# tugitbartlomiej/ViTParticleFilterTracker

Measured on AMD Instinct MI355X. Metric: frames/sec @ 4096 particles, ViT-B/16 224px; 1/2/4/8 MI355X scaling, higher is better.
Workload: dtype bf16; 1 GPU; 4096 particles, vit_base_patch16_224 bf16, 224x224 frames, full tracking step per frame; particles=4096, particles_per_gpu=4096, arch=vit_base_patch16_224, hip_graph=True, parallelism=particle-shard x1

## Files before the change

### include/vpf.h

```cpp
#ifndef VPF_H
#define VPF_H
#include <stddef.h>
#include <stdint.h>

#ifdef __cplusplus
extern "C" {
#endif

#define VPF_ERR_ARG (-1)

#define VPF_EPI_BIAS 0
#define VPF_EPI_BIAS_GELU 1
#define VPF_EPI_BIAS_RESIDUAL 2
#define VPF_EPI_PATCH 3
#define VPF_EPI_LN 4
#define VPF_EPI_LN_GELU 5

const char* vpf_version(void);

int vpf_predict(float* particles, int64_t n, int64_t ld, int64_t global_begin, uint64_t seed,
                uint32_t frame, float sig_x, float sig_y, float sig_s, float width, float height,
                float smin, float smax, void* stream);

int vpf_crop_patches_bf16(const uint8_t* frame, int H, int W, uint32_t* rgba_ws, const float* particles,
                          int64_t ld, int64_t n, float w0, float h0, int S, int patch, int Kp,
                          const float* norm_ab_host, uint16_t* out, void* stream);
int vpf_crop_patches_f32(const uint8_t* frame, int H, int W, uint32_t* rgba_ws, const float* particles,
                         int64_t ld, int64_t n, float w0, float h0, int S, int patch, int Kp,
                         const float* norm_ab_host, float* out, void* stream);

int vpf_cls_rows_bf16(uint16_t* tokens, int64_t n_part, int N, int D, const float* cls,
                      const float* pos, float* stats_out, int parts, void* stream);
int vpf_cls_rows_f32(float* tokens, int64_t n_part, int N, int D, const float* cls, const float* pos,
                     void* stream);

int vpf_gemm_bf16(const uint16_t* A, int64_t lda, const uint16_t* W, const float* bias,
                  const uint16_t* residual, const float* pos, int patch_rows, const float* row_stats,
                  const float* colsum, uint16_t* C, int64_t ldc, int64_t M, int64_t N, int64_t K,
                  int epilogue, int stats_parts, float ln_eps, float* stats_out, uint8_t* C8, int64_t ld8,
                  uint32_t* Cs, int64_t lds_c, void* stream);
int vpf_gemm_bf16_splitk(const uint16_t* A, int64_t lda, const uint16_t* W, const float* bias,
                         const uint16_t* residual, const float* row_stats, const float* colsum, uint16_t* C,
                         int64_t ldc, int64_t M, int64_t N, int64_t K, int epilogue, int splits, float* stats_out,
                         float* partial_ws, int64_t ws_elems, void* stream);
int vpf_gemm_tune(int kernel, int group);

int vpf_gemm_mx8(const uint8_t* A8, int64_t lda, const uint32_t* As, int64_t lds_a, const uint8_t* W8,
                 const uint32_t* Ws, const float* bias, const uint16_t* residual, const float* row_stats,
                 const float* colsum, uint16_t* C, int64_t ldc, uint8_t* C8, int64_t ld8, uint32_t* Cs,
                 int64_t lds_c, int64_t M, int64_t N, int64_t K, int epilogue, int stats_parts, float ln_eps,
                 float* stats_out, void* stream);
int vpf_quantize_mx8(const uint16_t* X, int64_t ldx, int64_t rows, int64_t K, int64_t out_stride, uint8_t* X8,
                     int64_t ld8, uint32_t* S, int64_t lds, void* stream);
int vpf_gemm_f32(const float* A, int64_t lda, const float* W, const float* bias, const float* residual,
                 const float* pos, int patch_rows, const float* row_stats, const float* colsum, float* C,
                 int64_t ldc, int64_t M, int64_t N, int64_t K, int epilogue, void* stream);

int vpf_row_stats_bf16(const uint16_t* x, int64_t rows, int D, int64_t x_stride, float eps, float* out,
                       void* stream);
int vpf_row_stats_f32(const float* x, int64_t rows, int D, int64_t x_stride, float eps, float* out,
                      void* stream);

int vpf_stats_combine(const float* planes, int parts, int64_t plane_stride, int64_t rows, int D, float eps, float* out,
                      void* stream);

int vpf_layernorm_bf16(const uint16_t* x, int64_t rows, int D, int64_t x_stride, const float* gamma,
                       const float* beta, float eps, uint16_t* y, int64_t y_stride, void* stream);
int vpf_layernorm_f32(const float* x, int64_t rows, int D, int64_t x_stride, const float* gamma,
                      const float* beta, float eps, float* y, int64_t y_stride, void* stream);

int vpf_attention_bf16(const uint16_t* qkv, uint16_t* out, int64_t B, int N, int H, int hd,
                       float scale, int q_rows, void* stream);
int vpf_attention_bf16_mx8(const uint16_t* qkv, int64_t B, int N, int H, int hd, float scale, uint8_t* out8,
                           int64_t ld8, uint32_t* s8, int64_t lds, void* stream);
int vpf_attention_f32(const float* qkv, float* out, int64_t B, int N, int H, int hd, float scale,
                      int q_rows, void* stream);
int vpf_head_gather_bf16(const uint16_t* Y, int64_t n, int H, int hd, uint16_t* out, int64_t ldo, void* stream);
int vpf_cls_attn_fold_bf16(const uint16_t* tokens, int64_t n_part, int N, int H, const float* planes,
                           int64_t plane_rows, float eps, const uint16_t* G, int64_t ldg, const uint16_t* q,
                           int64_t ldq, const float* bk, float scale, uint16_t* out, int64_t ldo, void* stream);

int vpf_cls_weight_bf16(const uint16_t* tokens, int64_t n, int N, int D, const float* gamma,
                        const float* beta, float eps, const float* tmpl, float lam, int bits,
                        float* feat_out, float* sim_out, int64_t* Q, void* stream);
int vpf_cls_weight_f32(const float* tokens, int64_t n, int N, int D, const float* gamma,
                       const float* beta, float eps, const float* tmpl, float lam, int bits,
                       float* feat_out, float* sim_out, int64_t* Q, void* stream);

int vpf_cosine_weight_f32(const float* feat, int64_t n, int D, const float* tmpl, float lam, int bits,
                          float* sim_out, int64_t* Q, void* stream);

int vpf_shard_stats(const int64_t* Q, const float* particles, int64_t ld, int64_t n, int64_t* out_T,
                    double* out_sums, void* stream);

int vpf_resample(const int64_t* Q, int64_t n_local, int64_t global_begin, int64_t offset,
                 int64_t total, int64_t P, uint32_t U, int uniform, int64_t slot_begin,
                 int64_t slot_end, const float* particles, int64_t ld, int32_t* anc_out,
                 float* states_out, int64_t out_ld, int64_t* cdf_ws, void* stream);

int vpf_estimate_resample(const int64_t* Q, int64_t q_stride, const float* particles, int64_t ld,
                          int64_t p_stride, int64_t n_shard, int64_t P, uint64_t seed, uint32_t frame,
                          int64_t slot_begin, int64_t slot_end, int32_t* anc_out, float* states_out,
                          int64_t out_ld, int64_t* cdf_ws, int64_t* stats_out, void* stream);

#define VPF_RESAMPLE_SYSTEMATIC 0
#define VPF_RESAMPLE_STRATIFIED 1

int vpf_weight_prior(int64_t* Q, const int64_t* carry, int64_t n, int bits, void* stream);

int vpf_estimate_resample_ex(const int64_t* Q, int64_t q_stride, const float* particles, int64_t ld,
                             int64_t p_stride, int64_t n_shard, int64_t P, uint64_t seed, uint32_t frame,
                             int64_t slot_begin, int64_t slot_end, int32_t* anc_out, float* states_out,
                             int64_t out_ld, int64_t* cdf_ws, int64_t* stats_out, int method, double ess_tau,
                             int bits, int64_t* carry_out, void* stream);

#ifdef __cplusplus
}
#endif
#endif
```

### vitparticlefiltertracker_amd/_lib.py

```python
from __future__ import annotations

import ctypes
import os
import subprocess
import threading

import torch

_HERE = os.path.dirname(os.path.abspath(__file__))
LIB_PATH = os.environ.get("VPF_LIB_PATH") or os.path.join(_HERE, "libvpf.so")
CSRC = os.path.join(_HERE, "csrc")

_lock = threading.Lock()
_lib = None

VPF_EPI_BIAS = 0
VPF_EPI_BIAS_GELU = 1
VPF_EPI_BIAS_RESIDUAL = 2
VPF_EPI_PATCH = 3
VPF_EPI_LN = 4
VPF_EPI_LN_GELU = 5
VPF_RESAMPLE_SYSTEMATIC = 0
VPF_RESAMPLE_STRATIFIED = 1

_P, _I64, _I32, _U64, _U32, _F32, _F64 = (ctypes.c_void_p, ctypes.c_int64, ctypes.c_int, ctypes.c_uint64,
                                          ctypes.c_uint32, ctypes.c_float, ctypes.c_double)

SIGNATURES = {
    "vpf_predict": [_P, _I64, _I64, _I64, _U64, _U32, _F32, _F32, _F32, _F32, _F32, _F32, _F32, _P],
    "vpf_crop_patches_bf16": [_P, _I32, _I32, _P, _P, _I64, _I64, _F32, _F32, _I32, _I32, _I32, _P, _P, _P],
    "vpf_crop_patches_f32": [_P, _I32, _I32, _P, _P, _I64, _I64, _F32, _F32, _I32, _I32, _I32, _P, _P, _P],
    "vpf_cls_rows_bf16": [_P, _I64, _I32, _I32, _P, _P, _P, _I32, _P],
    "vpf_cls_rows_f32": [_P, _I64, _I32, _I32, _P, _P, _P],
    "vpf_gemm_bf16": [_P, _I64, _P, _P, _P, _P, _I32, _P, _P, _P, _I64, _I64, _I64, _I64, _I32, _I32, _F32, _P,
                      _P, _I64, _P, _I64, _P],
    "vpf_gemm_mx8": [_P, _I64, _P, _I64, _P, _P, _P, _P, _P, _P, _P, _I64, _P, _I64, _P, _I64, _I64, _I64, _I64,
                     _I32, _I32, _F32, _P, _P],
    "vpf_quantize_mx8": [_P, _I64, _I64, _I64, _I64, _P, _I64, _P, _I64, _P],
    "vpf_gemm_bf16_splitk": [_P, _I64, _P, _P, _P, _P, _P, _P, _I64, _I64, _I64, _I64, _I32, _I32, _P, _P, _I64, _P],
    "vpf_gemm_tune": [_I32, _I32],
    "vpf_gemm_f32": [_P, _I64, _P, _P, _P, _P, _I32, _P, _P, _P, _I64, _I64, _I64, _I64, _I32, _P],
    "vpf_row_stats_bf16": [_P, _I64, _I32, _I64, _F32, _P, _P],
    "vpf_stats_combine": [_P, _I32, _I64, _I64, _I32, _F32, _P, _P],
    "vpf_row_stats_f32": [_P, _I64, _I32, _I64, _F32, _P, _P],
    "vpf_layernorm_bf16": [_P, _I64, _I32, _I64, _P, _P, _F32, _P, _I64, _P],
    "vpf_layernorm_f32": [_P, _I64, _I32, _I64, _P, _P, _F32, _P, _I64, _P],
    "vpf_attention_bf16": [_P, _P, _I64, _I32, _I32, _I32, _F32, _I32, _P],
    "vpf_attention_f32": [_P, _P, _I64, _I32, _I32, _I32, _F32, _I32, _P],
    "vpf_attention_bf16_mx8": [_P, _I64, _I32, _I32, _I32, _F32, _P, _I64, _P, _I64, _P],
    "vpf_head_gather_bf16": [_P, _I64, _I32, _I32, _P, _I64, _P],
    "vpf_cls_attn_fold_bf16": [_P, _I64, _I32, _I32, _P, _I64, _F32, _P, _I64, _P, _I64, _P, _F32, _P, _I64, _P],
    "vpf_cls_weight_bf16": [_P, _I64, _I32, _I32, _P, _P, _F32, _P, _F32, _I32, _P, _P, _P, _P],
    "vpf_cls_weight_f32": [_P, _I64, _I32, _I32, _P, _P, _F32, _P, _F32, _I32, _P, _P, _P, _P],
    "vpf_cosine_weight_f32": [_P, _I64, _I32, _P, _F32, _I32, _P, _P, _P],
    "vpf_shard_stats": [_P, _P, _I64, _I64, _P, _P, _P],
    "vpf_resample": [_P, _I64, _I64, _I64, _I64, _I64, _U32, _I32, _I64, _I64, _P, _I64, _P, _P, _I64, _P, _P],
    "vpf_estimate_resample": [_P, _I64, _P, _I64, _I64, _I64, _I64, _U64, _U32, _I64, _I64, _P, _P, _I64, _P, _P,
                              _P],
    "vpf_weight_prior": [_P, _P, _I64, _I32, _P],
    "vpf_estimate_resample_ex": [_P, _I64, _P, _I64, _I64, _I64, _I64, _U64, _U32, _I64, _I64, _P, _P, _I64, _P, _P,
                                 _I32, _F64, _I32, _P, _P],
}


class VPFError(RuntimeError):
    pass


def build(force: bool = False) -> str:
    args = ["make", "-s", "-C", CSRC, "-j8"]
    if force:
        subprocess.run(["make", "-s", "-C", CSRC, "clean"], check=True)
    subprocess.run(args, check=True)
    return LIB_PATH


def lib() -> ctypes.CDLL:
    global _lib
    if _lib is not None:
        return _lib
    with _lock:
        if _lib is None:
            if not os.path.exists(LIB_PATH):
                raise VPFError(f"libvpf.so not found at {LIB_PATH}; run `python -c 'import __graft_entry__ as g; "
                               f"g.build()'` (or `make -C {CSRC}`)")
            L = ctypes.CDLL(LIB_PATH, mode=ctypes.RTLD_GLOBAL)
            override = os.environ.get("VPF_LIB_PATH") is not None
            for name, argtypes in SIGNATURES.items():
                if override and not hasattr(L, name):
                    continue
                fn = getattr(L, name)
                fn.argtypes = argtypes
                fn.restype = ctypes.c_int
            L.vpf_version.argtypes = []
            L.vpf_version.restype = ctypes.c_char_p
            _lib = L
    return _lib


def check(rc: int, name: str) -> None:
    if rc != 0:
        if rc == -1:
            raise VPFError(f"{name}: argument violates the shape contract of include/vpf.h")
        raise VPFError(f"{name}: HIP error {rc}")


def stream_ptr(stream=None) -> int:
    s = stream if stream is not None else torch.cuda.current_stream()
    return s.cuda_stream


def ptr(t) -> int:
    return 0 if t is None else t.data_ptr()


def call(name: str, *args) -> None:
    check(getattr(lib(), name)(*args), name)
```

### vitparticlefiltertracker_amd/csrc/gemm_bf16.hip

```cpp
#include <algorithm>
#include "gemm_common.h"

using namespace vpf;
using namespace vpf::gemm;

namespace {

constexpr int BK = 64;
constexpr int OPERAND_BYTES = BM * BK * 2;
static_assert(OPERAND_BYTES == TILE_BYTES, "bf16 K-tile geometry");
constexpr int AUX_PARTS = 15;
constexpr int MAX_PARTS = 16;
constexpr int AUX_BYTES = 2048 + AUX_PARTS * 2048;

template <int EPI, bool WIDE = false, bool OUT8 = false, bool PART = false>
__global__ __launch_bounds__(NTHREADS) void k_gemm_bf16(const bf16_t* __restrict__ A, int lda,
                                                        const bf16_t* __restrict__ W,
                                                        const float* __restrict__ bias,
                                                        const bf16_t* residual,
                                                        const float* __restrict__ pos, int g2,
                                                        const float2* __restrict__ stats,
                                                        const float* __restrict__ colsum,
                                                        bf16_t* C, int ldc, int M, int N, int K, int group,
                                                        int stats_parts, float ln_eps, float* stats_out,
                                                        int stats_rows, Out8 o8) {
    constexpr int SMEM = 5 * OPERAND_BYTES;
    static_assert(AUX_BYTES <= OPERAND_BYTES, "aux region must fit the free A slot of the deep ring");
    __shared__ __attribute__((aligned(16))) char smem[SMEM];
    const int tid = threadIdx.x, lane = tid & 63;
    const int wid = __builtin_amdgcn_readfirstlane(tid >> 6);

    int m0, n0;
    tile_of(M, N, group, m0, n0);
    constexpr bool DIRECT = (EPI == VPF_EPI_LN_GELU || EPI == VPF_EPI_BIAS_GELU) && !OUT8 && !PART;

    const int kbase = PART ? (int)blockIdx.y * (K / (int)gridDim.y) : 0;
    const char* Ablk = reinterpret_cast<const char*>(A) + (size_t)m0 * lda * 2 + (size_t)kbase * 2;
    const char* Bblk = reinterpret_cast<const char*>(W) + (size_t)n0 * K * 2 + (size_t)kbase * 2;
    uint32_t offA[4], offB[4];
#pragma unroll
    for (int i = 0; i < 4; ++i) {
        const int g = i * 8 + wid;
        const int row = 8 * g + (lane >> 3);
        const int pch = lane & 7;
        const int lch = pch ^ ((row >> 1) & 7);
        const int ra = min(row, M - 1 - m0);
        const int rb = min(DIRECT ? wperm(row) : row, N - 1 - n0);
        offA[i] = (uint32_t)ra * (uint32_t)(lda * 2) + (uint32_t)(lch * 16);
        offB[i] = (uint32_t)rb * (uint32_t)(K * 2) + (uint32_t)(lch * 16);
    }
    auto stage_a = [&](int kt) {
        char* la = smem + (kt % 3) * OPERAND_BYTES;
        const uint32_t koff = (uint32_t)kt * (BK * 2);
#pragma unroll
        for (int i = 0; i < 4; ++i)
            __builtin_amdgcn_global_load_lds((gptr_t)(Ablk + offA[i] + koff), (lptr_t)(la + (i * 8 + wid) * 1024), 16, 0, 0);
    };
    auto stage_b = [&](int kt) {
        char* lb = smem + (3 + (kt & 1)) * OPERAND_BYTES;
        const uint32_t koff = (uint32_t)kt * (BK * 2);
#pragma unroll
        for (int i = 0; i < 4; ++i)
            __builtin_amdgcn_global_load_lds((gptr_t)(Bblk + offB[i] + koff), (lptr_t)(lb + (i * 8 + wid) * 1024), 16, 0, 0);
    };

    const int wm = wid >> 2, wn = wid & 3;
    f32x4 acc[4][8];
#pragma unroll
    for (int j = 0; j < 4; ++j)
#pragma unroll
        for (int i = 0; i < 8; ++i) acc[j][i] = f32x4{0.f, 0.f, 0.f, 0.f};

    const int fr = lane & 15, fq = lane >> 4;

    constexpr bool LN = (EPI == VPF_EPI_LN || EPI == VPF_EPI_LN_GELU) && !PART;
    const int nk = (PART ? K / (int)gridDim.y : K) / BK;
    char* aux = smem + (nk % 3) * OPERAND_BYTES;
    constexpr bool wide = LN && WIDE;
    char* planes_lds = wide ? smem + ((nk + 1) % 3) * OPERAND_BYTES : aux + 2048;
    auto load_planes = [&](char* dst) { dma_planes(dst, stats, stats_parts, m0, M, wid, opaque_lane()); };
    auto load_aux = [&]() {
        if constexpr (PART) return;
        dma_bias_colsum<LN>(aux, bias, colsum, n0, N, wid, opaque_lane());
// ... 130 lines not shown
    if constexpr (LN) dma_planes(aux + 2048, stats, stats_parts, m0, M, wid, lane);
    stage(0, 0); stage(1, 0); stage(2, 0); stage(3, 0); stage(0, 1); stage(1, 1);
    asm volatile("s_waitcnt vmcnt(8)" ::: "memory");
    __builtin_amdgcn_s_barrier();
    if (wm == 1) __builtin_amdgcn_s_barrier();
    asm volatile("" ::: "memory");

    f32x4 acc[4][8];
#pragma unroll
    for (int j = 0; j < 4; ++j)
#pragma unroll
        for (int i = 0; i < 8; ++i) acc[j][i] = f32x4{0.f, 0.f, 0.f, 0.f};

    const int fr = lane & 15, fq = lane >> 4;
    const int sw = (fr >> 1) & 7;
    const int abase = (wm * 64 + fr) * 128, bbase = (wn * 32 + fr) * 128;
    auto mfma_quadrant = [&](const i32x4 (&fa)[2][4], const i32x4 (&fb)[2][2], int mh, int nh) {
        asm volatile("s_waitcnt lgkmcnt(0)" ::: "memory");
        __builtin_amdgcn_sched_barrier(0);
#pragma unroll
        for (int ks = 0; ks < 2; ++ks)
#pragma unroll
            for (int j = 0; j < 2; ++j)
#pragma unroll
                for (int i = 0; i < 4; ++i)
                    acc[nh * 2 + j][mh * 4 + i] = __builtin_amdgcn_mfma_f32_16x16x32_bf16(
                        __builtin_bit_cast(bf16x8, fb[ks][j]), __builtin_bit_cast(bf16x8, fa[ks][i]),
                        acc[nh * 2 + j][mh * 4 + i], 0, 0, 0);
        __builtin_amdgcn_sched_barrier(0);
    };
    auto read_a = [&](i32x4 (&fa)[2][4], const char* slot) {
#pragma unroll
        for (int ks = 0; ks < 2; ++ks)
#pragma unroll
            for (int i = 0; i < 4; ++i) fa[ks][i] = lds16(slot + abase + i * 2048 + (((ks * 4 + fq) ^ sw) << 4));
    };
    auto read_b = [&](i32x4 (&fb)[2][2], const char* slot) {
#pragma unroll
        for (int ks = 0; ks < 2; ++ks)
#pragma unroll
            for (int j = 0; j < 2; ++j) fb[ks][j] = lds16(slot + bbase + j * 2048 + (((ks * 4 + fq) ^ sw) << 4));
    };
    auto bar = [&]() {
        __builtin_amdgcn_sched_barrier(0);
        __builtin_amdgcn_s_barrier();
        __builtin_amdgcn_sched_barrier(0);
    };

    for (int kt = 0; kt < nk; ++kt) {
        const char* buf = smem + (kt & 1) * 4 * HALF;
        i32x4 fa0[2][4], fa1[2][4], fb0[2][2], fb1[2][2];
        read_a(fa0, buf);
        read_b(fb0, buf + HALF);
        stage(2, kt + 1);
        asm volatile("s_waitcnt vmcnt(8)" ::: "memory");
        bar();
        mfma_quadrant(fa0, fb0, 0, 0);
        bar();
        read_b(fb1, buf + 2 * HALF);
        stage(3, kt + 1);
        asm volatile("s_waitcnt vmcnt(8)" ::: "memory");
        bar();
        mfma_quadrant(fa0, fb1, 0, 1);
        bar();
        read_a(fa1, buf + 3 * HALF);
        stage(0, kt + 2);
        bar();
        mfma_quadrant(fa1, fb1, 1, 1);
        bar();
        stage(1, kt + 2);
        asm volatile("s_waitcnt vmcnt(8)" ::: "memory");
        bar();
        mfma_quadrant(fa1, fb0, 1, 0);
        bar();
    }
    if (wm == 0) __builtin_amdgcn_s_barrier();
    asm volatile("s_waitcnt vmcnt(0)" ::: "memory");

    if constexpr (LN) combine_planes(aux + 2048, aux, stats_parts, K, ln_eps, tid);
    finish_tile<EPI, OUT8, DIRECT>(smem + wid * 16384, aux, acc, wm, wn, m0, n0, lane, residual, pos, g2, C, ldc, M, N,
                                   stats_out, stats_rows, o8);
}

}

#define VPF_IS_LN(E) ((E) == VPF_EPI_LN || (E) == VPF_EPI_LN_GELU)
#define VPF_IS_PROD(E) ((E) == VPF_EPI_BIAS_RESIDUAL || (E) == VPF_EPI_PATCH)
#define VPF_GEMM_ARGS                                                                                        \
    A, (int)lda, W, bias, residual, pos, patch_rows, reinterpret_cast<const float2*>(row_stats), colsum, C,     \
        (int)ldc, m, n, k, group, stats_parts, ln_eps, stats_out, stats_rows, o8
#define VPF_GEMM_LAUNCH(E)                                                                                   \
    do {                                                                                                     \
        if (kern == 5 && !(VPF_IS_LN(E) && stats_parts > AUX_PARTS) && o8.q == nullptr)                      \
            hipLaunchKernelGGL((k_gemm_pp<E, false>), grid, block, 0, s, VPF_GEMM_ARGS);                     \
        else if (kern == 5 && VPF_IS_PROD(E) && o8.q != nullptr)                                             \
            hipLaunchKernelGGL((k_gemm_pp<E, VPF_IS_PROD(E)>), grid, block, 0, s, VPF_GEMM_ARGS);            \
        else if (VPF_IS_LN(E) && stats_parts > AUX_PARTS)                                                    \
            hipLaunchKernelGGL((k_gemm_bf16<E, VPF_IS_LN(E)>), grid, block, 0, s, VPF_GEMM_ARGS);             \
        else if (VPF_IS_PROD(E) && o8.q != nullptr)                                                          \
            hipLaunchKernelGGL((k_gemm_bf16<E, false, VPF_IS_PROD(E)>), grid, block, 0, s, VPF_GEMM_ARGS);    \
        else                                                                                                 \
            hipLaunchKernelGGL((k_gemm_bf16<E>), grid, block, 0, s, VPF_GEMM_ARGS);                           \
    } while (0)

constexpr int kDefaultGroup = 4;
static int g_kernel = 0;
static int g_group = -1;
static int gemm_kernel_for(int epilogue) {
    if (g_kernel) return g_kernel;
    return (epilogue == VPF_EPI_LN || epilogue == VPF_EPI_LN_GELU) ? 5 : 1;
}
static int tile_group_for(int64_t N, int epilogue) {
    if (g_group >= 0) return g_group;
    if (N <= 1024) return 2;
    return epilogue == VPF_EPI_LN_GELU ? 8 : kDefaultGroup;
}
int vpf_gemm_tile_group() { return g_group >= 0 ? g_group : kDefaultGroup; }
int vpf_gemm_tile_group_mx8(int epilogue) {
    if (g_group >= 0) return g_group;
    return epilogue == VPF_EPI_LN ? 8 : kDefaultGroup;
}
VPF_API int vpf_gemm_tune(int kernel, int group) {
    if (kernel != 0 && kernel != 1 && kernel != 5) return VPF_ERR_ARG;
    if (group < -1 || group > 64) return VPF_ERR_ARG;
    g_kernel = kernel;
    g_group = kernel == 0 ? -1 : group;
    return 0;
}

int vpf_check_out8(const uint8_t* C8, int64_t ld8, const uint32_t* Cs, int64_t lds_c, int64_t rows, int64_t N) {
    if (!C8) return Cs ? VPF_ERR_ARG : 0;
    if (!Cs || N % 128 != 0 || ld8 < N || ld8 % 8 != 0 || ((uintptr_t)C8 & 7) || lds_c < rows || lds_c % 64 != 0 ||
        ((uintptr_t)Cs & 3) || ld8 > INT32_MAX || lds_c > INT32_MAX / 4)
        return VPF_ERR_ARG;
    return 0;
}

int64_t vpf_gemm_check(int64_t M, int64_t N, int64_t K, int64_t k_unit, int64_t lda, int a_align, int a_bytes,
                       bool has_c, int64_t ldc, const float* bias, const float* colsum, const float* row_stats) {
    if (M <= 0 || N <= 0 || K <= 0 || K % k_unit != 0 || N % 8 != 0 || lda < K || lda % a_align != 0) return 0;
    if (has_c && (ldc < N || ldc % 8 != 0 || ldc > INT32_MAX / 2)) return 0;
    if (M > INT32_MAX / 2 || N > 65536 || K > 65536 || lda > INT32_MAX / 2) return 0;
    if ((uint64_t)BM * (uint64_t)lda * (uint64_t)a_bytes > UINT32_MAX) return 0;
    if (((uintptr_t)bias & 15) || ((uintptr_t)colsum & 15) || ((uintptr_t)row_stats & 7)) return 0;
    const int64_t tiles = ((M + BM - 1) / BM) * ((N + BN - 1) / BN);
    return tiles > INT32_MAX ? 0 : tiles;
}

VPF_API int vpf_gemm_bf16(const uint16_t* A, int64_t lda, const uint16_t* W, const float* bias,
                          const uint16_t* residual, const float* pos, int patch_rows, const float* row_stats,
                          const float* colsum, uint16_t* C, int64_t ldc, int64_t M, int64_t N, int64_t K,
                          int epilogue, int stats_parts, float ln_eps, float* stats_out, uint8_t* C8, int64_t ld8,
                          uint32_t* Cs, int64_t lds_c, void* stream) {
    const int64_t tiles = vpf_gemm_check(M, N, K, BK, lda, 8, 2, true, ldc, bias, colsum, row_stats);
    if (!tiles) return VPF_ERR_ARG;
    if (!A || !W || !bias || !C) return VPF_ERR_ARG;
    if (epilogue == VPF_EPI_BIAS_RESIDUAL && !residual) return VPF_ERR_ARG;
    if (epilogue == VPF_EPI_PATCH && (!pos || patch_rows <= 0 || M % patch_rows != 0)) return VPF_ERR_ARG;
    if ((epilogue == VPF_EPI_LN || epilogue == VPF_EPI_LN_GELU) && (!row_stats || !colsum)) return VPF_ERR_ARG;
    if (stats_parts < 0 || stats_parts > MAX_PARTS || !(ln_eps >= 0.f)) return VPF_ERR_ARG;
    if (stats_out && (((uintptr_t)stats_out & 7) || (epilogue != VPF_EPI_BIAS_RESIDUAL && epilogue != VPF_EPI_PATCH)))
        return VPF_ERR_ARG;
    const int64_t srows = epilogue == VPF_EPI_PATCH ? (M / patch_rows) * (patch_rows + 1) : M;
    if (srows > INT32_MAX) return VPF_ERR_ARG;
    const int stats_rows = (int)srows;
    if (C8 && epilogue != VPF_EPI_BIAS_RESIDUAL && epilogue != VPF_EPI_PATCH) return VPF_ERR_ARG;
    if (vpf_check_out8(C8, ld8, Cs, lds_c, srows, N)) return VPF_ERR_ARG;
    const Out8 o8{C8, reinterpret_cast<uint8_t*>(Cs), (int)ld8, (int)lds_c};
    hipStream_t s = (hipStream_t)stream;
    const dim3 grid((unsigned)tiles), block(NTHREADS);
    const int kern = gemm_kernel_for(epilogue);
    const int group = tile_group_for(N, epilogue);
    const int m = (int)M, n = (int)N, k = (int)K;
    switch (epilogue) {
        case VPF_EPI_BIAS: VPF_GEMM_LAUNCH(VPF_EPI_BIAS); break;
        case VPF_EPI_BIAS_GELU: VPF_GEMM_LAUNCH(VPF_EPI_BIAS_GELU); break;
        case VPF_EPI_BIAS_RESIDUAL: VPF_GEMM_LAUNCH(VPF_EPI_BIAS_RESIDUAL); break;
        case VPF_EPI_PATCH: VPF_GEMM_LAUNCH(VPF_EPI_PATCH); break;
        case VPF_EPI_LN: VPF_GEMM_LAUNCH(VPF_EPI_LN); break;
        case VPF_EPI_LN_GELU: VPF_GEMM_LAUNCH(VPF_EPI_LN_GELU); break;
        default: return VPF_ERR_ARG;
    }
    VPF_RETURN_LAUNCH();
}

template <int EPI>
__global__ __launch_bounds__(256) void k_splitk_reduce(const float* __restrict__ P, int S, int M, int N,
                                                       const float* __restrict__ bias,
                                                       const float2* __restrict__ stats,
                                                       const float* __restrict__ colsum, const bf16_t* residual,
                                                       bf16_t* C, int64_t ldc, float* stats_out) {
    constexpr bool LN = (EPI == VPF_EPI_LN || EPI == VPF_EPI_LN_GELU);
    constexpr bool GELU = (EPI == VPF_EPI_BIAS_GELU || EPI == VPF_EPI_LN_GELU);
    const int per_row = N >> 3;
    const int64_t t = (int64_t)blockIdx.x * blockDim.x + threadIdx.x;
    const bool live = t < (int64_t)M * per_row;
    const int m = live ? (int)(t / per_row) : 0;
    const int n = live ? (int)(t - (int64_t)m * per_row) * 8 : 0;
    float v[8];
    if (live) {
        const float* p = P + (size_t)m * N + n;
        const float4 a0 = *reinterpret_cast<const float4*>(p), a1 = *reinterpret_cast<const float4*>(p + 4);
        v[0] = a0.x; v[1] = a0.y; v[2] = a0.z; v[3] = a0.w; v[4] = a1.x; v[5] = a1.y; v[6] = a1.z; v[7] = a1.w;
        for (int s = 1; s < S; ++s) {
            const float* q = p + (size_t)s * M * N;
            const float4 b0 = *reinterpret_cast<const float4*>(q), b1 = *reinterpret_cast<const float4*>(q + 4);
            v[0] += b0.x; v[1] += b0.y; v[2] += b0.z; v[3] += b0.w; v[4] += b1.x; v[5] += b1.y; v[6] += b1.z; v[7] += b1.w;
        }
        float rstd = 1.f, nrm = 0.f;
        if constexpr (LN) {
            const float2 st = stats[m];
            rstd = st.y;
            nrm = -st.y * st.x;
        }
#pragma unroll
        for (int e = 0; e < 8; ++e) {
            float y = LN ? fmaf(rstd, v[e], fmaf(nrm, colsum[n + e], bias[n + e])) : v[e] + bias[n + e];
            if constexpr (GELU) {
                const f32x2 g = gelu_sig2(f32x2{y, y});
                y = g.x;
            }
            v[e] = y;
        }
    }
    uint32_t o[4];
#pragma unroll
    for (int e = 0; e < 4; ++e) o[e] = pack_bf2(v[2 * e], v[2 * e + 1]);
    if constexpr (EPI == VPF_EPI_BIAS_RESIDUAL) {
        if (live) {
            const uint4 v = add_bf16x8(make_uint4(o[0], o[1], o[2], o[3]),
                                       *reinterpret_cast<const uint4*>(residual + (size_t)m * ldc + n));
            o[0] = v.x; o[1] = v.y; o[2] = v.z; o[3] = v.w;
        }
        if (stats_out != nullptr) {
            float s1 = 0.f, s2 = 0.f;
            if (live) {
#pragma unroll
                for (int e = 0; e < 4; ++e) {
                    const float lo = bf2f((bf16_t)(o[e] & 0xffff)), hi = bf2f((bf16_t)(o[e] >> 16));
                    s1 += lo + hi;
                    s2 = fmaf(lo, lo, s2);
                    s2 = fmaf(hi, hi, s2);
                }
            }
#pragma unroll
            for (int x = 1; x < 8; x <<= 1) {
                s1 += __shfl_xor(s1, x, 64);
                s2 += __shfl_xor(s2, x, 64);
            }
            if (live && (n & 63) == 0)
                *reinterpret_cast<float2*>(stats_out + ((int64_t)(n >> 6) * M + m) * 2) = make_float2(s1, s2);
        }
    }
    if (live) *reinterpret_cast<uint4*>(C + (size_t)m * ldc + n) = make_uint4(o[0], o[1], o[2], o[3]);
}

// ... 46 lines not shown
```

### vitparticlefiltertracker_amd/csrc/gemm_common.h

```cpp
#pragma once
#include "vpf_common.h"
#include "mx8.h"
#include "../../include/vpf.h"

int vpf_gemm_tile_group();
int vpf_gemm_tile_group_mx8(int epilogue);
int vpf_check_out8(const uint8_t* C8, int64_t ld8, const uint32_t* Cs, int64_t lds_c, int64_t rows, int64_t N);
int64_t vpf_gemm_check(int64_t M, int64_t N, int64_t K, int64_t k_unit, int64_t lda, int a_align, int a_bytes,
                       bool has_c, int64_t ldc, const float* bias, const float* colsum, const float* row_stats);

namespace vpf {
namespace gemm {

typedef const __attribute__((address_space(1))) void* gptr_t;
typedef __attribute__((address_space(3))) void* lptr_t;
typedef short bf16x8 __attribute__((ext_vector_type(8)));
typedef int i32x4 __attribute__((ext_vector_type(4)));

__device__ __forceinline__ i32x4 lds16(const char* p) {
    i32x4 v;
    asm volatile("ds_read_b128 %0, %1" : "=v"(v) : "v"((uint32_t)(uintptr_t)(lptr_t)p));
    return v;
}
__device__ __forceinline__ int lds4(const void* p) {
    int v;
    asm volatile("ds_read_b32 %0, %1" : "=v"(v) : "v"((uint32_t)(uintptr_t)(lptr_t)p));
    return v;
}
__device__ __forceinline__ int opaque_lane() {
    int l;
    asm volatile("v_mbcnt_lo_u32_b32 %0, -1, 0\n\tv_mbcnt_hi_u32_b32 %0, -1, %0" : "=v"(l));
    return l;
}
typedef float f32x4 __attribute__((ext_vector_type(4)));
typedef float f32x2 __attribute__((ext_vector_type(2)));

constexpr int BM = 256, BN = 256;
constexpr int NTHREADS = 512;
constexpr int TILE_BYTES = BM * 128;

typedef unsigned u32x4_nt __attribute__((ext_vector_type(4)));
__device__ __forceinline__ void st16_nt(void* p, uint4 v) {
    __builtin_nontemporal_store(u32x4_nt{v.x, v.y, v.z, v.w}, reinterpret_cast<u32x4_nt*>(p));
}

__device__ __forceinline__ void tile_of_lid(int M, int N, int group, int lid, int& m0, int& n0) {
    const int tiles_n = (N + BN - 1) / BN;
    int tm, tn;
    if (group > 0) {
        const int tiles_m = (M + BM - 1) / BM;
        const int per_group = group * tiles_n;
        const int g = lid / per_group, idx = lid - g * per_group;
        const int gm0 = g * group;
        const int gsz = min(group, tiles_m - gm0);
        tn = idx / gsz;
        tm = gm0 + (idx - tn * gsz);
    } else {
        tm = lid / tiles_n;
        tn = lid - tm * tiles_n;
    }
    m0 = tm * BM;
    n0 = tn * BN;
}
__device__ __forceinline__ int xcd_first(int nwg, int xcd) {
    const int q = nwg >> 3, r = nwg & 7;
    return xcd < r ? xcd * (q + 1) : r * (q + 1) + (xcd - r) * q;
}
__device__ __forceinline__ void tile_of(int M, int N, int group, int& m0, int& n0) {
    const int nwg = gridDim.x, bid = blockIdx.x;
    tile_of_lid(M, N, group, xcd_first(nwg, bid & 7) + (bid >> 3), m0, n0);
}

__device__ __forceinline__ f32x2 gelu_sig2(f32x2 x) {
    constexpr float L2E = 1.4426950408889634f;
    constexpr float c1 = -1.6003141571059616f * L2E, c2 = -0.06940178687219423f * L2E;
    const f32x2 q = (x * x) * c2 + c1;
    const f32x2 t = x * q;
    const f32x2 d = f32x2{__builtin_amdgcn_exp2f(t.x), __builtin_amdgcn_exp2f(t.y)} + 1.0f;
    return x * f32x2{__builtin_amdgcn_rcpf(d.x), __builtin_amdgcn_rcpf(d.y)};
}

struct Out8 {
    uint8_t* q;
    uint8_t* s;
    int ldq, lds;
};

constexpr bool epi_is_ln(int epi) { return epi == VPF_EPI_LN || epi == VPF_EPI_LN_GELU; }
constexpr bool epi_is_gelu(int epi) { return epi == VPF_EPI_BIAS_GELU || epi == VPF_EPI_LN_GELU; }

template <bool LN>
__device__ __forceinline__ void dma_bias_colsum(char* aux, const float* __restrict__ bias,
                                                const float* __restrict__ colsum, int n0, int N, int wid, int lane) {
    if (wid == 0)
        __builtin_amdgcn_global_load_lds((gptr_t)(bias + min(n0 + lane * 4, N - 4)), (lptr_t)aux, 16, 0, 0);
    if constexpr (LN) {
        if (wid == 1)
            __builtin_amdgcn_global_load_lds((gptr_t)(colsum + min(n0 + lane * 4, N - 4)), (lptr_t)(aux + 1024), 16, 0, 0);
    }
}
__device__ __forceinline__ void dma_planes(char* dst, const float2* __restrict__ stats, int stats_parts, int m0, int M,
                                           int wid, int lane) {
    const float* sd = reinterpret_cast<const float*>(stats);
    const int planes = stats_parts > 0 ? stats_parts : 1;
    if ((M & 1) == 0 && ((uintptr_t)sd & 15) == 0) {
        for (int pc = wid; pc < 2 * planes; pc += 8) {
            const int p = pc >> 1, hf = pc & 1;
            __builtin_amdgcn_global_load_lds(
                (gptr_t)(sd + (int64_t)p * 2 * M + min(2 * m0 + hf * 256 + lane * 4, 2 * M - 4)),
                (lptr_t)(dst + p * 2048 + hf * 1024), 16, 0, 0);
        }
    } else {
        for (int p = 0; p < planes; ++p)
            __builtin_amdgcn_global_load_lds(
                (gptr_t)(sd + (int64_t)p * 2 * M + min(2 * m0 + wid * 64 + lane, 2 * M - 1)),
                (lptr_t)(dst + p * 2048 + wid * 256), 4, 0, 0);
    }
}
__device__ __forceinline__ void combine_planes(const char* planes_lds, char* aux, int stats_parts, int K, float ln_eps,
                                               int tid) {
    if (stats_parts > 0 && tid < BM) {
        float sm = 0.f, sq = 0.f;
        for (int p = 0; p < stats_parts; ++p) {
            const float2 st = *reinterpret_cast<const float2*>(planes_lds + p * 2048 + tid * 8);
            sm += st.x;
            sq += st.y;
        }
        const float inv_k = 1.0f / (float)K;
        const float mean = sm * inv_k;
        const float var = fmaxf(fmaf(sq, inv_k, -mean * mean), 0.f);
        *reinterpret_cast<float2*>(aux + 2048 + tid * 8) = make_float2(mean, __builtin_amdgcn_rsqf(var + ln_eps));
    }
}

struct EpiCols { float4 b, c; };
struct EpiRow { f32x2 rstd, nrm; };
struct Frag4 { f32x2 lo, hi; };
template <bool LN>
__device__ __forceinline__ EpiCols epi_cols(const char* aux, int col) {
    EpiCols v;
    v.b = *reinterpret_cast<const float4*>(aux + col * 4);
    v.c = LN ? *reinterpret_cast<const float4*>(aux + 1024 + col * 4) : make_float4(0.f, 0.f, 0.f, 0.f);
    return v;
}
template <bool LN>
__device__ __forceinline__ EpiRow epi_row(const char* aux, int row) {
    if constexpr (LN) {
        const float2 st = *reinterpret_cast<const float2*>(aux + 2048 + row * 8);
        return EpiRow{f32x2{st.y, st.y}, f32x2{-st.y * st.x, -st.y * st.x}};
    } else {
        return EpiRow{f32x2{1.f, 1.f}, f32x2{0.f, 0.f}};
    }
}
// ... 393 lines not shown
```

Baseline: 7.550 frames/s.

## Add wide 256x384 bf16 GEMM kernel for the residual FC2 projection

Adds a new GEMM kernel with a 256x384 output tile and a double-buffered LDS ring that fills 160 KB. It uses software-pipelined LDS reads interleaved with MFMA and a bias+residual epilogue that can also emit row stats. It becomes the default for the bias+residual epilogue when N=768, K=3072 and M is large, which is the ViT MLP down-projection. The goal is more operand reuse per tile and fewer tiles for N=768, at the cost of lower occupancy and a more fragile hand-scheduled pipeline.

```diff
diff --git a/include/vpf.h b/include/vpf.h
--- a/include/vpf.h
+++ b/include/vpf.h
@@ -44,6 +44,7 @@
                          int64_t ldc, int64_t M, int64_t N, int64_t K, int epilogue, int splits, float* stats_out,
                          float* partial_ws, int64_t ws_elems, void* stream);
 int vpf_gemm_tune(int kernel, int group);
+int vpf_gemm_kernel_for(int epilogue, int64_t M, int64_t N, int64_t K, int has_fp8);
 
 int vpf_gemm_mx8(const uint8_t* A8, int64_t lda, const uint32_t* As, int64_t lds_a, const uint8_t* W8,
                  const uint32_t* Ws, const float* bias, const uint16_t* residual, const float* row_stats,
diff --git a/vitparticlefiltertracker_amd/_lib.py b/vitparticlefiltertracker_amd/_lib.py
--- a/vitparticlefiltertracker_amd/_lib.py
+++ b/vitparticlefiltertracker_amd/_lib.py
@@ -39,6 +39,7 @@
     "vpf_quantize_mx8": [_P, _I64, _I64, _I64, _I64, _P, _I64, _P, _I64, _P],
     "vpf_gemm_bf16_splitk": [_P, _I64, _P, _P, _P, _P, _P, _P, _I64, _I64, _I64, _I64, _I32, _I32, _P, _P, _I64, _P],
     "vpf_gemm_tune": [_I32, _I32],
+    "vpf_gemm_kernel_for": [_I32, _I64, _I64, _I64, _I32],
     "vpf_gemm_f32": [_P, _I64, _P, _P, _P, _P, _I32, _P, _P, _P, _I64, _I64, _I64, _I64, _I32, _P],
     "vpf_row_stats_bf16": [_P, _I64, _I32, _I64, _F32, _P, _P],
     "vpf_stats_combine": [_P, _I32, _I64, _I64, _I32, _F32, _P, _P],
diff --git a/vitparticlefiltertracker_amd/csrc/gemm_bf16.hip b/vitparticlefiltertracker_amd/csrc/gemm_bf16.hip
--- a/vitparticlefiltertracker_amd/csrc/gemm_bf16.hip
+++ b/vitparticlefiltertracker_amd/csrc/gemm_bf16.hip
@@ -1,4 +1,6 @@
 #include <algorithm>
+#include <type_traits>
+#include <utility>
 #include "gemm_common.h"
 
 using namespace vpf;
@@ -295,6 +297,217 @@
                                    stats_out, stats_rows, o8);
 }
 
+constexpr int WBN = 384;
+constexpr int WIDE_A_BYTES = BM * BK * 2, WIDE_W_BYTES = WBN * BK * 2;
+
+template <int OFF>
+__device__ __forceinline__ i32x4 lds16o(uint32_t addr) {
+    i32x4 v;
+    asm volatile("ds_read_b128 %0, %1 offset:%2" : "=v"(v) : "v"(addr), "n"(OFF));
+    return v;
+}
+template <int... Is, class F>
+__device__ __forceinline__ void static_for(std::integer_sequence<int, Is...>, F&& f) {
+    (f(std::integral_constant<int, Is>{}), ...);
+}
+template <int CNT>
+__device__ __forceinline__ void wait_lds() {
+    asm volatile("s_waitcnt lgkmcnt(%0)" ::"n"(CNT) : "memory");
+    __builtin_amdgcn_sched_barrier(0);
+}
+
+__global__ __launch_bounds__(NTHREADS) void k_gemm_wide(const bf16_t* __restrict__ A, int lda,
+                                                        const bf16_t* __restrict__ W,
+                                                        const float* __restrict__ bias, const bf16_t* residual,
+                                                        bf16_t* C, int ldc, int M, int N, int K, int group,
+                                                        float* stats_out, int stats_rows) {
+    constexpr int SMEM = 2 * WIDE_A_BYTES + 2 * WIDE_W_BYTES;
+    static_assert(SMEM == 160 * 1024, "the wide ring fills the LDS");
+    __shared__ __attribute__((aligned(128))) char smem[SMEM];
+    const int tid = threadIdx.x, lane = tid & 63;
+    const int wid = __builtin_amdgcn_readfirstlane(tid >> 6);
+    const int wm = wid >> 1, wn = wid & 1;
+
+    int m0, n0;
+    tile_of<WBN>(M, N, group, m0, n0);
+
+    const char* Ablk = reinterpret_cast<const char*>(A) + (size_t)m0 * lda * 2;
+    const char* Bblk = reinterpret_cast<const char*>(W) + (size_t)n0 * K * 2;
+    const int lrow = 8 * wid + (lane >> 3);
+    const uint32_t lch16 = (uint32_t)(((lane & 7) ^ ((lrow >> 1) & 7)) * 16);
+    uint32_t offA[4];
+#pragma unroll
+    for (int i = 0; i < 4; ++i) offA[i] = (uint32_t)min(lrow + 64 * i, M - 1 - m0) * (uint32_t)(lda * 2) + lch16;
+    const uint32_t offB = (uint32_t)lrow * (uint32_t)(K * 2) + lch16;
+    const size_t strideB = (size_t)64 * K * 2;
+    auto stage_a1 = [&](int kt, int i) {
+        const char* base = Ablk + (uint32_t)kt * (BK * 2);
+        asm volatile("" : "+s"(base));
+        __builtin_amdgcn_global_load_lds((gptr_t)(base + offA[i]),
+                                         (lptr_t)(smem + (kt & 1) * WIDE_A_BYTES + (i * 8 + wid) * 1024), 16, 0, 0);
+    };
+    auto stage_b1 = [&](int kt, int i) {
+        const char* base = Bblk + i * strideB + (uint32_t)kt * (BK * 2);
+        asm volatile("" : "+s"(base));
+        __builtin_amdgcn_global_load_lds((gptr_t)(base + offB),
+                                         (lptr_t)(smem + 2 * WIDE_A_BYTES + (kt & 1) * WIDE_W_BYTES + (i * 8 + wid) * 1024),
+                                         16, 0, 0);
+    };
+
+    f32x4 acc[12][4];
+#pragma unroll
+    for (int j = 0; j < 12; ++j)
+#pragma unroll
+        for (int i = 0; i < 4; ++i) acc[j][i] = f32x4{0.f, 0.f, 0.f, 0.f};
+
+    const int fr = lane & 15, fq = lane >> 4;
+    const uint32_t fch = (uint32_t)((fq ^ ((fr >> 1) & 7)) << 4);
+    const uint32_t fa0 = (uint32_t)(uintptr_t)(lptr_t)smem + (uint32_t)((wm * 64 + fr) * 128) + fch;
+    const uint32_t fb0 = (uint32_t)(uintptr_t)(lptr_t)smem + (uint32_t)(2 * WIDE_A_BYTES + (wn * 192 + fr) * 128) + fch;
+
+    const int nk = K / BK;
+    char* aux = smem + (nk & 1) * WIDE_A_BYTES;
+
+    int klast = nk - 1;
+    asm volatile("" : "+s"(klast));
+    auto kstep = [&](int kt) {
+        asm volatile("s_waitcnt vmcnt(0)" ::: "memory");
+        __builtin_amdgcn_s_barrier();
+        asm volatile("" ::: "memory");
+        if (kt == klast) {
+            const int lane = opaque_lane();
+            if (wid == 0)
+                __builtin_amdgcn_global_load_lds((gptr_t)(bias + min(n0 + lane * 4, N - 4)), (lptr_t)aux, 16, 0, 0);
+            if (wid == 1)
+                __builtin_amdgcn_global_load_lds((gptr_t)(bias + min(n0 + 256 + lane * 4, N - 4)), (lptr_t)(aux + 1024), 16,
+                                                 0, 0);
+        }
+        const uint32_t ra = fa0 + (uint32_t)((kt & 1) * WIDE_A_BYTES), rb = fb0 + (uint32_t)((kt & 1) * WIDE_W_BYTES);
+        i32x4 a[4], b[3][2];
+        auto read_a = [&](int ks) {
+            const uint32_t p = ra ^ (uint32_t)(ks * 64);
+            a[0] = lds16o<0>(p); a[1] = lds16o<2048>(p); a[2] = lds16o<4096>(p); a[3] = lds16o<6144>(p);
+        };
+        auto read_b = [&](auto nc) {
+            constexpr int n = decltype(nc)::value, g = n % 6;
+            const uint32_t p = rb ^ (uint32_t)((n / 6) * 64);
+            b[n % 3][0] = lds16o<2 * g * 2048>(p);
+            b[n % 3][1] = lds16o<(2 * g + 1) * 2048>(p);
+        };
+        read_a(0);
+        read_b(std::integral_constant<int, 0>{});
+        read_b(std::integral_constant<int, 1>{});
+        static_for(std::make_integer_sequence<int, 12>{}, [&](auto nc) {
+            constexpr int n = decltype(nc)::value, g = n % 6;
+            if constexpr (n + 2 < 12) read_b(std::integral_constant<int, n + 2>{});
+            wait_lds<(n == 6 || n == 10) ? 2 : n == 11 ? 0 : 4>();
+            if constexpr (n < 4) stage_a1(min(kt + 1, klast), n);
+            else if constexpr (n < 10) stage_b1(min(kt + 1, klast), n - 4);
+#pragma unroll
+            for (int jj = 0; jj < 2; ++jj)
+#pragma unroll
+                for (int i = 0; i < 4; ++i)
+                    acc[2 * g + jj][i] = __builtin_amdgcn_mfma_f32_16x16x32_bf16(
+                        __builtin_bit_cast(bf16x8, b[n % 3][jj]), __builtin_bit_cast(bf16x8, a[i]), acc[2 * g + jj][i], 0,
+                        0, 0);
+            if constexpr (n == 5) {
+                __builtin_amdgcn_sched_barrier(0);
+                read_a(1);
+            }
+        });
+    };
+
+    stage_b1(0, 0); stage_b1(0, 1); stage_b1(0, 2); stage_b1(0, 3); stage_b1(0, 4); stage_b1(0, 5);
+    stage_a1(0, 0); stage_a1(0, 1); stage_a1(0, 2); stage_a1(0, 3);
+    for (int kt = 0; kt < nk; ++kt) kstep(kt);
+    __builtin_amdgcn_sched_barrier(0);
+
+    __builtin_amdgcn_s_waitcnt(0x0F70);
+    const int mw = m0 + wm * 64, nw = n0 + wn * 192;
+    char* img = smem + ((nk & 1) ^ 1) * WIDE_A_BYTES + wid * 2048;
+    char* park = smem + 2 * WIDE_A_BYTES + wid * 12288;
+    uint4 res[12][2];
+    auto load_res = [&](int u) {
+        const int i = u / 3, p = u % 3, ll = opaque_lane();
+        const int m = mw + i * 16 + 2 * (ll >> 3), n = nw + p * 64 + (ll & 7) * 8;
+        const bf16_t* rl = residual + (int64_t)m * ldc + n;
+#pragma unroll
+        for (int h = 0; h < 2; ++h)
+            res[u][h] = (m + h < M && n < N) ? *reinterpret_cast<const uint4*>(rl + (int64_t)h * ldc)
+                                             : make_uint4(0, 0, 0, 0);
+    };
+    load_res(0);
+    load_res(1);
+    load_res(2);
+    epilogue_barrier();
+    const EpiRow rw1 = epi_row<false>(aux, 0);
+    const bool want_stats = stats_out != nullptr;
+#pragma unroll
+    for (int i = 0; i < 4; ++i) {
+#pragma unroll
+        for (int p = 0; p < 3; ++p) {
+            const int ul = opaque_lane();
+            const int efr = ul & 15, efq = ul >> 4, c16 = ul & 7, r8 = ul >> 3;
+#pragma unroll
+            for (int j = 0; j < 4; ++j) {
+                const EpiCols cl = epi_cols<false>(aux, wn * 192 + (p * 4 + j) * 16 + efq * 4);
+                epi_to_image4<VPF_EPI_BIAS_RESIDUAL>(img, efr, j * 4 + efq, acc[p * 4 + j][i], cl, rw1);
+            }
+            __builtin_amdgcn_wave_barrier();
+            const int n = nw + p * 64 + c16 * 8;
+            bf16_t* Cl = C + (int64_t)(mw + i * 16 + 2 * r8) * ldc + n;
+#pragma unroll
+            for (int h = 0; h < 2; ++h) {
+                const int row = 2 * r8 + h;
+                uint4 v = image_get16(img, row, c16, h == 1);
+                const bool ok = mw + i * 16 + row < M && n < N;
+                v = add_bf16x8(v, res[i * 3 + p][h]);
+                if (want_stats) {
+                    typedef __bf16 bf16x2_t __attribute__((ext_vector_type(2)));
+                    const uint32_t w[4] = {v.x, v.y, v.z, v.w};
+                    const bf16x2_t one2 = __builtin_bit_cast(bf16x2_t, 0x3F803F80u);
+                    float s1 = 0.f, s2 = 0.f;
+#pragma unroll
+                    for (int e = 0; e < 4; ++e) {
+                        const bf16x2_t pr = __builtin_bit_cast(bf16x2_t, w[e]);
+                        s1 = __builtin_amdgcn_fdot2_f32_bf16(pr, one2, s1, false);
+                        s2 = __builtin_amdgcn_fdot2_f32_bf16(pr, pr, s2, false);
+                    }
+                    if (!ok) { s1 = 0.f; s2 = 0.f; }
+                    *reinterpret_cast<float2*>(park + (p * 64 + i * 16 + row) * 64 + c16 * 8) = make_float2(s1, s2);
+                }
+                if (ok) *reinterpret_cast<uint4*>(Cl + (int64_t)h * ldc) = v;
+            }
+            if (i * 3 + p + 3 < 12) load_res(i * 3 + p + 3);
+            __builtin_amdgcn_wave_barrier();
+            __builtin_amdgcn_sched_barrier(0);
+        }
+    }
+    if (want_stats) {
+        __builtin_amdgcn_wave_barrier();
+#pragma unroll
+        for (int rd = 0; rd < 2; ++rd) {
+            const int task = rd * 64 + opaque_lane(), p = task >> 5, l = task & 31;
+            const int nb = nw + p * 64;
+            if (p < 3 && nb < N) {
+                const char* src = park + (p * 64 + 2 * l) * 64;
+                float4 t = make_float4(0.f, 0.f, 0.f, 0.f);
+#pragma unroll
+                for (int q = 0; q < 4; ++q) {
+                    const float4 u0 = *reinterpret_cast<const float4*>(src + q * 16);
+                    const float4 u1 = *reinterpret_cast<const float4*>(src + 64 + q * 16);
+                    t.x += u0.x + u0.z; t.y += u0.y + u0.w;
+                    t.z += u1.x + u1.z; t.w += u1.y + u1.w;
+                }
+                float* plane = stats_out + (int64_t)(nb >> 6) * stats_rows * 2;
+                const int m = mw + 2 * l;
+                if (m + 1 < M) *reinterpret_cast<float4*>(plane + (int64_t)m * 2) = t;
+                else if (m < M) *reinterpret_cast<float2*>(plane + (int64_t)m * 2) = make_float2(t.x, t.y);
+            }
+        }
+    }
+}
+
 }
 
 #define VPF_IS_LN(E) ((E) == VPF_EPI_LN || (E) == VPF_EPI_LN_GELU)
@@ -317,10 +530,18 @@
     } while (0)
 
 constexpr int kDefaultGroup = 4;
+constexpr int kWideKernel = 11;
 static int g_kernel = 0;
 static int g_group = -1;
-static int gemm_kernel_for(int epilogue) {
-    if (g_kernel) return g_kernel;
+static bool wide_applies(int epilogue, int64_t N, bool out8) {
+    return epilogue == VPF_EPI_BIAS_RESIDUAL && !out8 && N % WBN == 0 && N <= 1024;
+}
+static bool wide_is_default(int64_t M, int64_t N, int64_t K) { return N == 768 && K == 3072 && M >= 262144; }
+static int gemm_kernel_for(int epilogue, int64_t M, int64_t N, int64_t K, bool out8) {
+    const bool applies = wide_applies(epilogue, N, out8);
+    if (g_kernel == kWideKernel && applies) return kWideKernel;
+    if (g_kernel && g_kernel != kWideKernel) return g_kernel;
+    if (applies && wide_is_default(M, N, K)) return kWideKernel;
     return (epilogue == VPF_EPI_LN || epilogue == VPF_EPI_LN_GELU) ? 5 : 1;
 }
 static int tile_group_for(int64_t N, int epilogue) {
@@ -333,8 +554,11 @@
     if (g_group >= 0) return g_group;
     return epilogue == VPF_EPI_LN ? 8 : kDefaultGroup;
 }
+VPF_API int vpf_gemm_kernel_for(int epilogue, int64_t M, int64_t N, int64_t K, int has_fp8) {
+    return gemm_kernel_for(epilogue, M, N, K, has_fp8 != 0);
+}
 VPF_API int vpf_gemm_tune(int kernel, int group) {
-    if (kernel != 0 && kernel != 1 && kernel != 5) return VPF_ERR_ARG;
+    if (kernel != 0 && kernel != 1 && kernel != 5 && kernel != kWideKernel) return VPF_ERR_ARG;
     if (group < -1 || group > 64) return VPF_ERR_ARG;
     g_kernel = kernel;
     g_group = kernel == 0 ? -1 : group;
@@ -382,9 +606,15 @@
     const Out8 o8{C8, reinterpret_cast<uint8_t*>(Cs), (int)ld8, (int)lds_c};
     hipStream_t s = (hipStream_t)stream;
     const dim3 grid((unsigned)tiles), block(NTHREADS);
-    const int kern = gemm_kernel_for(epilogue);
+    const int kern = gemm_kernel_for(epilogue, M, N, K, C8 != nullptr);
     const int group = tile_group_for(N, epilogue);
     const int m = (int)M, n = (int)N, k = (int)K;
+    if (kern == kWideKernel) {
+        const dim3 wgrid((unsigned)(((M + BM - 1) / BM) * (N / WBN)));
+        hipLaunchKernelGGL(k_gemm_wide, wgrid, block, 0, s, A, (int)lda, W, bias, residual, C, (int)ldc, m, n, k, group,
+                           stats_out, stats_rows);
+        VPF_RETURN_LAUNCH();
+    }
     switch (epilogue) {
         case VPF_EPI_BIAS: VPF_GEMM_LAUNCH(VPF_EPI_BIAS); break;
         case VPF_EPI_BIAS_GELU: VPF_GEMM_LAUNCH(VPF_EPI_BIAS_GELU); break;
diff --git a/vitparticlefiltertracker_amd/csrc/gemm_common.h b/vitparticlefiltertracker_amd/csrc/gemm_common.h
--- a/vitparticlefiltertracker_amd/csrc/gemm_common.h
+++ b/vitparticlefiltertracker_amd/csrc/gemm_common.h
@@ -44,7 +44,9 @@
     __builtin_nontemporal_store(u32x4_nt{v.x, v.y, v.z, v.w}, reinterpret_cast<u32x4_nt*>(p));
 }
 
+template <int TBN = BN>
 __device__ __forceinline__ void tile_of_lid(int M, int N, int group, int lid, int& m0, int& n0) {
+    constexpr int BN = TBN;
     const int tiles_n = (N + BN - 1) / BN;
     int tm, tn;
     if (group > 0) {
@@ -66,9 +68,10 @@
     const int q = nwg >> 3, r = nwg & 7;
     return xcd < r ? xcd * (q + 1) : r * (q + 1) + (xcd - r) * q;
 }
+template <int TBN = BN>
 __device__ __forceinline__ void tile_of(int M, int N, int group, int& m0, int& n0) {
     const int nwg = gridDim.x, bid = blockIdx.x;
-    tile_of_lid(M, N, group, xcd_first(nwg, bid & 7) + (bid >> 3), m0, n0);
+    tile_of_lid<TBN>(M, N, group, xcd_first(nwg, bid & 7) + (bid >> 3), m0, n0);
 }
 
 __device__ __forceinline__ f32x2 gelu_sig2(f32x2 x) {
```

Result: no change. 7.624 frames/s (median of 6 runs) (+1.0%).
